# wfus/Fully-Homomorphic-Image-Processing

Hardware: AMD Instinct MI355X
Metric: encrypted 8x8 blocks/sec (homomorphic DCT+quant) (higher is better)
Workload: dtype f64

## Files before the change

fully-homomorphic-image-processing_amd/csrc/dct_fused.hip:

```cpp
#include "internal.h"

#include <cstdlib>

#include "fp64_core.h"

#pragma clang fp contract(off)

namespace {
using namespace fp64;

template <int L, int LE> struct Shape {
    static constexpr int N = 1 << L, E = 1 << LE, TP = N >> LE, NP = (L + LE - 1) / LE, LDS_WORDS = N + (N >> LE);
};
__host__ __device__ constexpr int g_lo(int L, int LE, int p) { return (L - LE * p - LE) < 0 ? 0 : (L - LE * p - LE); }
__host__ __device__ constexpr int g_stages(int L, int LE, int p) { return (L - LE * p) > LE ? LE : (L - LE * p); }
template <int LO, int LE> __device__ __forceinline__ int g_index(int tid, int r) {
    return ((tid >> LO) << (LO + LE)) | (r << LO) | (tid & ((1 << LO) - 1));
}
template <int LO, int LE> __device__ __forceinline__ int g_pad(int j) { return j + ((j >> (LO + LE)) << LO); }

template <int L, int LE, int P> struct PassTw {
    static constexpr int LO = g_lo(L, LE, P), S = g_stages(L, LE, P), NTW = (1 << LE) - 1;
    static constexpr int rb(int u) { return (L - 1 - (LE * P + u)) - LO; }
    static constexpr int count(int u) { return 1 << (LE - 1 - rb(u)); }
    static constexpr int offset(int u) { int o = 0; for (int v = 0; v < u; v++) o += count(v); return o; }
};
template <int L, int LE, int P>
__device__ __forceinline__ void load_tw(double (&w)[(1 << LE) - 1], const double *__restrict__ tw, int tid) {
    using T = PassTw<L, LE, P>;
    const int th = (P == 0) ? 0 : (tid >> T::LO);
#pragma unroll
    for (int u = 0; u < T::S; u++) {
#pragma unroll
        for (int i = 0; i < T::count(u); i++) w[T::offset(u) + i] = tw[(1 << (LE * P + u)) + ((th << (LE - 1 - T::rb(u))) | i)];
    }
}

template <int L, int LE, int P, int M>
__device__ __forceinline__ void fwd_pass(double (&x)[M][1 << LE], const double (&w)[(1 << LE) - 1], double p, double pinv) {
    using T = PassTw<L, LE, P>;
    constexpr int E = 1 << LE, KB = (LE == 3) ? 2 : 1;
#pragma unroll
    for (int u = 0; u < T::S; u++) {
        const int rb = T::rb(u);
#pragma unroll
        for (int b0 = 0; b0 < E / 2; b0 += KB) {
            double t[KB * M], wm[KB * M];
#pragma unroll
            for (int kb = 0; kb < KB; kb++) {
                const int b = b0 + kb, r0 = ((b >> rb) << (rb + 1)) | (b & ((1 << rb) - 1)), r1 = r0 | (1 << rb);
                const double wv = w[T::offset(u) + (r0 >> (rb + 1))];
#pragma unroll
                for (int m = 0; m < M; m++) { t[kb * M + m] = x[m][r1]; wm[kb * M + m] = wv; }
            }
            mmv<KB * M>(t, wm, p, pinv);
#pragma unroll
            for (int kb = 0; kb < KB; kb++) {
                const int b = b0 + kb, r0 = ((b >> rb) << (rb + 1)) | (b & ((1 << rb) - 1)), r1 = r0 | (1 << rb);
#pragma unroll
                for (int m = 0; m < M; m++) {
                    const double X = x[m][r0];
                    x[m][r0] = X + t[kb * M + m];
                    x[m][r1] = X - t[kb * M + m];
                }
            }
        }
    }
}

template <int L, int LE, int P, int M>
__device__ __forceinline__ void inv_pass(double (&x)[M][1 << LE], const double (&w)[(1 << LE) - 1], double ninv, double p, double pinv) {
    using T = PassTw<L, LE, P>;
    constexpr int E = 1 << LE, KB = (LE == 3) ? 2 : 1;
#pragma unroll
    for (int u = T::S - 1; u >= 0; u--) {
        const int sigma = LE * P + u, rb = T::rb(u);
        if (sigma == 0) {
#pragma unroll
            for (int b = 0; b < E / 2; b++) {
                const int r0 = ((b >> rb) << (rb + 1)) | (b & ((1 << rb) - 1)), r1 = r0 | (1 << rb);
                const double wv = w[T::offset(u) + (r0 >> (rb + 1))];
                double t[2 * M], wm[2 * M];
#pragma unroll
                for (int m = 0; m < M; m++) {
                    const double X = x[m][r0], Y = x[m][r1];
                    t[m] = X + Y; wm[m] = ninv;
                    t[M + m] = X - Y; wm[M + m] = wv;
                }
                mmv<2 * M>(t, wm, p, pinv);
#pragma unroll
                for (int m = 0; m < M; m++) { x[m][r0] = t[m]; x[m][r1] = t[M + m]; }
            }
        } else {
#pragma unroll
            for (int b0 = 0; b0 < E / 2; b0 += KB) {
                double t[KB * M], wm[KB * M];
#pragma unroll
                for (int kb = 0; kb < KB; kb++) {
                    const int b = b0 + kb, r0 = ((b >> rb) << (rb + 1)) | (b & ((1 << rb) - 1)), r1 = r0 | (1 << rb);
                    const double wv = w[T::offset(u) + (r0 >> (rb + 1))];
#pragma unroll
                    for (int m = 0; m < M; m++) {
                        const double X = x[m][r0], Y = x[m][r1];
                        x[m][r0] = X + Y;
                        t[kb * M + m] = X - Y; wm[kb * M + m] = wv;
                    }
                }
                mmv<KB * M>(t, wm, p, pinv);
#pragma unroll
                for (int kb = 0; kb < KB; kb++) {
                    const int b = b0 + kb, r0 = ((b >> rb) << (rb + 1)) | (b & ((1 << rb) - 1)), r1 = r0 | (1 << rb);
#pragma unroll
                    for (int m = 0; m < M; m++) x[m][r1] = t[kb * M + m];
                }
            }
        }
    }
}

template <int L, int LE, int LO_FROM, int LO_TO, int M>
__device__ __forceinline__ void transpose(double (&x)[M][1 << LE], double *lds, int tid, int &phase) {
    constexpr int PL = imin(LO_FROM, LO_TO), E = 1 << LE;
    constexpr bool WAVE_LOCAL = (Shape<L, LE>::TP <= 64) || (LO_FROM <= 6 && LO_TO <= 6);
#pragma unroll
    for (int m = 0; m < M; m++) {
        double *buf = lds + (phase & 1) * Shape<L, LE>::LDS_WORDS;
        phase++;
#pragma unroll
        for (int r = 0; r < E; r++) buf[g_pad<PL, LE>(g_index<LO_FROM, LE>(tid, r))] = x[m][r];
        if constexpr (WAVE_LOCAL) {
            __builtin_amdgcn_fence(__ATOMIC_RELEASE, "wavefront");
            __builtin_amdgcn_wave_barrier();
            __builtin_amdgcn_fence(__ATOMIC_ACQUIRE, "wavefront");
        } else {
            __syncthreads();
        }
#pragma unroll
        for (int r = 0; r < E; r++) x[m][r] = buf[g_pad<PL, LE>(g_index<LO_TO, LE>(tid, r))];
    }
}

template <int L, int LE, int M, typename PRE, int P = 0>
__device__ __forceinline__ void ntt_fwd(double (&x)[M][1 << LE], double (&w)[(1 << LE) - 1], const double *__restrict__ tw, double p, double pinv,
                                        double *lds, int tid, int &phase, PRE pre) {
    if constexpr (P + 1 < Shape<L, LE>::NP) {
        double wn[(1 << LE) - 1];
        if (LE >= 4) load_tw<L, LE, P + 1>(wn, tw, tid);
        fwd_pass<L, LE, P, M>(x, w, p, pinv);
        if (LE < 4) load_tw<L, LE, P + 1>(wn, tw, tid);
        if constexpr (P + 2 == Shape<L, LE>::NP) pre();
        transpose<L, LE, g_lo(L, LE, P), g_lo(L, LE, P + 1), M>(x, lds, tid, phase);
        ntt_fwd<L, LE, M, PRE, P + 1>(x, wn, tw, p, pinv, lds, tid, phase, pre);
    } else {
        fwd_pass<L, LE, P, M>(x, w, p, pinv);
    }
}
template <int L, int LE, int M, bool BIG, int P = Shape<L, LE>::NP - 1>
__device__ __forceinline__ void ntt_inv(double (&x)[M][1 << LE], double (&w)[(1 << LE) - 1], const double *__restrict__ itw, double p, double pinv,
                                        double *lds, int tid, int &phase) {
    if constexpr (P > 0) {
        double wn[(1 << LE) - 1];
        if (LE >= 4) load_tw<L, LE, P - 1>(wn, itw, tid);
        inv_pass<L, LE, P, M>(x, w, 0.0, p, pinv);
        if (LE < 4) load_tw<L, LE, P - 1>(wn, itw, tid);
        if constexpr (BIG) {
#pragma unroll
            for (int m = 0; m < M; m++)
#pragma unroll
                for (int r = 0; r < (1 << LE); r++) x[m][r] = red(x[m][r], p, pinv);
        }
        transpose<L, LE, g_lo(L, LE, P), g_lo(L, LE, P - 1), M>(x, lds, tid, phase);
        ntt_inv<L, LE, M, BIG, P - 1>(x, wn, itw, p, pinv, lds, tid, phase);
    } else {
        inv_pass<L, LE, P, M>(x, w, itw[0], p, pinv);
    }
}

constexpr double PACK_BIAS = 6755399441055744.0;
template <int E, int TP>
__device__ __forceinline__ void store_packed(char *__restrict__ ob, u32 vo, u32 so, const double (&x)[E]) {
    static_assert(E == 8, "packed layout is defined for 8 values per thread");
    u32 lo[8], hi[8];
#pragma unroll
    for (int r = 0; r < 8; r++) {
        const double t = x[r] + PACK_BIAS;
        lo[r] = (u32)__double2loint(t);
        hi[r] = (u32)__double2hiint(t);
    }
    u32 h[2];
#pragma unroll
    for (int g = 0; g < 2; g++) {
        const u32 p01 = __builtin_amdgcn_perm(hi[4 * g + 1], hi[4 * g + 0], 0x0c0c0400u);
        const u32 p23 = __builtin_amdgcn_perm(hi[4 * g + 3], hi[4 * g + 2], 0x0c0c0400u);
        h[g] = __builtin_amdgcn_perm(p23, p01, 0x05040100u);
    }
#pragma unroll
    for (int q = 0; q < 4; q++) *(u64 *)(ob + (size_t)(so + (q >> 1) * TP * 16 + (q & 1) * 8) + 2 * vo) = (u64)lo[2 * q] | ((u64)lo[2 * q + 1] << 32);
    *(u64 *)(ob + (size_t)(so + 4 * TP * 8) + vo) = (u64)h[0] | ((u64)h[1] << 32);
}
typedef __attribute__((address_space(3))) void lc_lptr;
template <int NT>
__device__ __forceinline__ void stage_consts(gwin_t w, u32 voff, u32 soff, u32 cstride_bytes, double *stg) {
#pragma unroll
    for (int i0 = 0; i0 < NT; i0 += 2) {
        const int i = (i0 + 1 < NT) ? i0 : NT - 2;
        __builtin_amdgcn_raw_ptr_buffer_load_lds(w, (lc_lptr *)(stg + i * 64), 16, voff, soff + (u32)i * cstride_bytes, 0, 0);
    }
}

template <int L, int LE, bool BIG, int HALF, bool PACK, bool LDSC>
__device__ __forceinline__ void rows_body(const u64 *__restrict__ in, double *__restrict__ mid, const double *__restrict__ consts,
                                          const double *__restrict__ tw, const Work &wk, double p, double pinv, u32 k, double *lds) {
    using SH = Shape<L, LE>;
    constexpr int N = SH::N, TP = SH::TP, E = SH::E, NC = HalfC<HALF>::NC, FIRST = HalfC<HALF>::FIRST;
    const int tid = threadIdx.x;
    const size_t poly_words = (size_t)k * N, ct_words = 2 * poly_words;
    const size_t base = ((size_t)wk.blk * 64 + 8 * wk.line) * ct_words + (size_t)wk.poly * poly_words + (size_t)wk.prime * N;
    const gwin_t win_in = gwin(in + base), win_mid = gwin(mid + base);
    const u32 vo = (u32)tid * 8u, ctb = (u32)(ct_words * 8);
    double w0[E - 1];
    load_tw<L, LE, 0>(w0, tw, tid);
    double x[4][E];
    u64 ra[2][E], rb[2][E];
    auto issue = [&](int m) {
#pragma unroll
        for (int r = 0; r < E; r++) {
            ra[m & 1][r] = gld_u64(win_in, vo, (u32)m * ctb + r * TP * 8);
            rb[m & 1][r] = gld_u64(win_in, vo, (u32)(7 - m) * ctb + r * TP * 8);
        }
    };
    auto combine = [&](int m) {
#pragma unroll
        for (int r = 0; r < E; r++) {
            const u64 A = ra[m & 1][r], B = rb[m & 1][r];
            x[m][r] = HALF ? u52_biased(A) - u52_biased(B) : u52_to_f64(A + B);
        }
    };
    if constexpr (LE >= 4) {
        issue(0);
        issue(1);
        asm volatile("" ::: "memory");
        combine(0);
        issue(2);
        asm volatile("" ::: "memory");
        combine(1);
        issue(3);
        asm volatile("" ::: "memory");
        combine(2);
        combine(3);
    } else {
#pragma unroll
        for (int m = 0; m < 4; m++) {
            issue(m);
            combine(m);
            asm volatile("" ::: "memory");
        }
    }
    const size_t cstride = (size_t)k * N;
    const gwin_t win_c = gwin(consts + (size_t)FIRST * cstride + (size_t)wk.prime * N);
    const u32 csb = (u32)(cstride * 8);
    double cn[9];
    auto fetch = [&](int r) {
#pragma unroll
        for (int i = 0; i < NC; i++) cn[i] = gld_f64(win_c, vo, (u32)i * csb + r * TP * 8);
    };
    int phase = 0;
    ntt_fwd<L, LE, 4>(x, w0, tw, p, pinv, lds, tid, phase, [&] { if (LE >= 4) fetch(0); });
    const int lane = tid & 63;
    double *stg = lds + (tid >> 6) * (2 * NC * 64);
    const u32 svoff = (u32)(((size_t)(lane >> 5) * cstride + (tid & ~63) + 2 * (lane & 31)) * sizeof(double));
    constexpr int NDMA = (NC + 1) / 2;
    if constexpr (LDSC) {
        __builtin_amdgcn_sched_barrier(0);
        __syncthreads();
        stage_consts<NC>(win_c, svoff, 0, csb, stg);
    }
#pragma unroll
    for (int r = 0; r < E; r++) {
        double c[9];
        if constexpr (LDSC) {
            if (r + 1 < E) stage_consts<NC>(win_c, svoff, (r + 1) * TP * 8, csb, stg + ((r + 1) & 1) * NC * 64);
            if (r + 1 < E) asm volatile("s_waitcnt vmcnt(%0)" ::"n"(NDMA) : "memory");
            else asm volatile("s_waitcnt vmcnt(0)" ::: "memory");
            const double *sr = stg + (r & 1) * NC * 64 + lane;
#pragma unroll
            for (int i = 0; i < NC; i++) c[i] = sr[i * 64];
        } else {
        if (LE < 4) fetch(r);
#pragma unroll
        for (int i = 0; i < NC; i++) c[i] = cn[i];
        if (LE >= 4 && r + 1 < E) fetch(r + 1);
        }
        line_half<HALF>(x[0][r], x[1][r], x[2][r], x[3][r], c, p, pinv);
        if (BIG) {
#pragma unroll
            for (int m = 0; m < 4; m++) x[m][r] = red(x[m][r], p, pinv);
        } else if (PACK && HALF == 0) {
            x[0][r] = red(x[0][r], p, pinv);
            x[2][r] = red(x[2][r], p, pinv);
        }
        if constexpr (LDSC) asm volatile("" ::"v"(x[0][r]), "v"(x[1][r]), "v"(x[2][r]), "v"(x[3][r]) : "memory");
    }
#pragma unroll
    for (int m = 0; m < 4; m++) {
        const u32 so = (u32)(2 * m + HALF) * ctb;
        if constexpr (PACK) {
            store_packed<E, TP>((char *)(mid + base), vo, so, x[m]);
        } else {
            if constexpr (LE >= 4) {
#pragma unroll
                for (int r = 0; r < E; r++) gst_f64(win_mid, 2 * vo, so + (r >> 1) * TP * 16 + (r & 1) * 8, x[m][r]);
            } else {
#pragma unroll
                for (int j = 0; j < E / 2; j++) gst_f64x2(win_mid, 2 * vo, so + j * TP * 16, x[m][2 * j], x[m][2 * j + 1]);
            }
        }
    }
}

__host__ __device__ constexpr int occ_waves(int tp, int lds_words) {
    return ((2 * lds_words * 16 <= 160 * 1024) ? 2 : 1) * tp / 256 < 1 ? 1 : ((2 * lds_words * 16 <= 160 * 1024) ? 2 : 1) * tp / 256;
}
template <int L, int LE> struct Occ { static constexpr int W = occ_waves(Shape<L, LE>::TP, Shape<L, LE>::LDS_WORDS); };

template <int L, int LE, bool BIG, bool PACK, bool LDSC>
__global__ __launch_bounds__((Shape<L, LE>::TP), (Occ<L, LE>::W)) void k_dct_rows(const u64 *__restrict__ in, double *__restrict__ mid,
                                                                  const double *__restrict__ consts, const double *__restrict__ tw_all,
                                                                  const Modulus *__restrict__ mods, u32 k) {
    __shared__ double lds[2 * Shape<L, LE>::LDS_WORDS];
    const Work wk = decode(blockIdx.x, k);
    const double p = (double)mods[wk.prime].q, pinv = 1.0 / p;
    const double *tw = tw_all + (size_t)wk.prime * Shape<L, LE>::N;
    if (wk.half) rows_body<L, LE, BIG, 1, PACK, LDSC>(in, mid, consts, tw, wk, p, pinv, k, lds);
    else rows_body<L, LE, BIG, 0, PACK, LDSC>(in, mid, consts, tw, wk, p, pinv, k, lds);
}

template <int L, int LE, bool BIG, int HALF, bool PACK>
__device__ __forceinline__ void cols_body(const double *__restrict__ mid, u64 *__restrict__ out, const double *__restrict__ consts,
                                          const double *__restrict__ cpairs, const double *__restrict__ itw, const Work &wk, double p, double pinv, u32 k, double *lds) {
    using SH = Shape<L, LE>;
    constexpr int N = SH::N, TP = SH::TP, E = SH::E, NC = HalfC<HALF>::NC, FIRST = HalfC<HALF>::FIRST;
    constexpr int LASTP = SH::NP - 1;
    const int tid = threadIdx.x;
    const size_t poly_words = (size_t)k * N, ct_words = 2 * poly_words;
    const size_t base = ((size_t)wk.blk * 64 + wk.line) * ct_words + (size_t)wk.poly * poly_words + (size_t)wk.prime * N;
    const size_t cstride = (size_t)k * N;
    const gwin_t win_mid = gwin(mid + base), win_out = gwin(out + base);
    const gwin_t win_c = PACK ? gwin(cpairs + 2 * ((size_t)(HALF ? 1 : 0) * cstride + (size_t)wk.prime * N))
                              : gwin(consts + (size_t)FIRST * cstride + (size_t)wk.prime * N);
    const gwin_t win_s = PACK ? gwin(cpairs + 2 * ((size_t)(DCT_NPAIR_LINE + 2 * (2 * wk.line + HALF)) * cstride + (size_t)wk.prime * N))
                              : gwin(consts + (size_t)(12 + 8 * HALF + wk.line) * cstride + (size_t)wk.prime * N);
    const gwin_t win_1 = gwin(consts + (size_t)(FIRST + NC - 1) * cstride + (size_t)wk.prime * N);
    const u32 vo = (u32)tid * 8u, rsb = (u32)(ct_words * 64), csb = (u32)(cstride * 8);
    const double pbias = p + 4503599627370496.0;
    double cn[9], sn[4];
    auto fetch = [&](int r) {
        if constexpr (PACK) {
#pragma unroll
            for (int i = 0; i < NC / 2; i++) {
                const f64x2 v = gld_f64x2(win_c, 2 * vo, (u32)i * 2 * csb + r * TP * 16);
                cn[2 * i] = v.a;
                cn[2 * i + 1] = v.b;
            }
            cn[NC - 1] = gld_f64(win_1, vo, r * TP * 8);
#pragma unroll
            for (int g = 0; g < 2; g++) {
                const f64x2 v = gld_f64x2(win_s, 2 * vo, (u32)g * 2 * csb + r * TP * 16);
                sn[2 * g] = v.a;
                sn[2 * g + 1] = v.b;
            }
        } else {
#pragma unroll
            for (int i = 0; i < NC; i++) cn[i] = gld_f64(win_c, vo, (u32)i * csb + r * TP * 8);
#pragma unroll
            for (int m = 0; m < 4; m++) sn[m] = gld_f64(win_s, vo, (u32)(16 * m) * csb + r * TP * 8);
        }
    };
    double wl[E - 1];
    if constexpr (!PACK) {
        fetch(0);
        load_tw<L, LE, LASTP>(wl, itw, tid);
    }
    double x[4][E];
    if constexpr (PACK) {
        u32x4 qa[4][2], qb[4][2];
        u64 ha[4], hb[4];
#pragma unroll
        for (int m = 0; m < 4; m++) {
#pragma unroll
            for (int g = 0; g < 2; g++) {
                qa[m][g] = gld_b128(win_mid, 2 * vo, (u32)m * rsb + g * TP * 16);
                qb[m][g] = gld_b128(win_mid, 2 * vo, (u32)(7 - m) * rsb + g * TP * 16);
            }
            ha[m] = gld_u64(win_mid, vo, (u32)m * rsb + 4 * TP * 8);
            hb[m] = gld_u64(win_mid, vo, (u32)(7 - m) * rsb + 4 * TP * 8);
        }
#pragma unroll
        for (int m = 0; m < 4; m++) {
#pragma unroll
            for (int r = 0; r < E; r++) {
                const u32 hwa = (r & 4) ? (u32)(ha[m] >> 32) : (u32)ha[m], hwb = (r & 4) ? (u32)(hb[m] >> 32) : (u32)hb[m];
                const double ta = __hiloint2double((int)(0x43380000u + (u32)(int)(signed char)(hwa >> (8 * (r & 3)))), (int)qa[m][r >> 2][r & 3]);
                const double tb = __hiloint2double((int)(0x43380000u + (u32)(int)(signed char)(hwb >> (8 * (r & 3)))), (int)qb[m][r >> 2][r & 3]);
                x[m][r] = HALF ? ta - tb : ta + (tb - 2.0 * PACK_BIAS);
            }
        }
    } else {
#pragma unroll
        for (int m = 0; m < 4; m++) {
#pragma unroll
            for (int j = 0; j < E / 2; j++) {
                const f64x2 A = gld_f64x2(win_mid, 2 * vo, (u32)m * rsb + j * TP * 16), B = gld_f64x2(win_mid, 2 * vo, (u32)(7 - m) * rsb + j * TP * 16);
                x[m][2 * j] = HALF ? A.a - B.a : A.a + B.a;
                x[m][2 * j + 1] = HALF ? A.b - B.b : A.b + B.b;
            }
        }
    }
#pragma unroll
    for (int r = 0; r < E; r++) {
        double c[9], sc[4];
        if (PACK) fetch(r);
#pragma unroll
        for (int i = 0; i < NC; i++) c[i] = cn[i];
#pragma unroll
        for (int m = 0; m < 4; m++) sc[m] = sn[m];
        if (!PACK && r + 1 < E) fetch(r + 1);
        line_half<HALF>(x[0][r], x[1][r], x[2][r], x[3][r], c, p, pinv);
        double y[4] = {x[0][r], x[1][r], x[2][r], x[3][r]};
        mmv<4>(y, sc, p, pinv);
#pragma unroll
        for (int m = 0; m < 4; m++) x[m][r] = y[m];
    }
    if constexpr (PACK) load_tw<L, LE, LASTP>(wl, itw, tid);
    int phase = 0;
    ntt_inv<L, LE, 4, BIG>(x, wl, itw, p, pinv, lds, tid, phase);
#pragma unroll
    for (int m = 0; m < 4; m++) {
#pragma unroll
        for (int r = 0; r < E; r++) gst_u64(win_out, vo, (u32)(2 * m + HALF) * rsb + r * TP * 8, f64_to_residue(x[m][r], pbias));
    }
}

template <int L, int LE, bool BIG, bool PACK>
__global__ __launch_bounds__((Shape<L, LE>::TP), (Occ<L, LE>::W)) void k_dct_cols(const double *__restrict__ mid, u64 *__restrict__ out,
                                                                  const double *__restrict__ consts, const double *__restrict__ cpairs, const double *__restrict__ itw_all,
                                                                  const Modulus *__restrict__ mods, u32 k) {
    __shared__ double lds[2 * Shape<L, LE>::LDS_WORDS];
    const Work wk = decode(blockIdx.x, k);
    const double p = (double)mods[wk.prime].q, pinv = 1.0 / p;
    const double *itw = itw_all + (size_t)wk.prime * Shape<L, LE>::N;
    if (wk.half) cols_body<L, LE, BIG, 1, PACK>(mid, out, consts, cpairs, itw, wk, p, pinv, k, lds);
    else cols_body<L, LE, BIG, 0, PACK>(mid, out, consts, cpairs, itw, wk, p, pinv, k, lds);
}

template <int L, int LE>
__global__ __launch_bounds__((Shape<L, LE>::TP), (Occ<L, LE>::W)) void k_dct_one_launch(const u64 *__restrict__ in, double *__restrict__ mid, u64 *__restrict__ out,
                                                                        const double *__restrict__ consts, const double *__restrict__ cpairs, const double *__restrict__ tw_all,
                                                                        const double *__restrict__ itw_all, const Modulus *__restrict__ mods, u32 k,
                                                                        u32 n_blocks, u32 dist, u32 *__restrict__ arrived, u32 *__restrict__ err) {
    __shared__ double lds[2 * Shape<L, LE>::LDS_WORDS];
    const u32 xcd = blockIdx.x & 7, seq = blockIdx.x >> 3, chunk = seq >> 5, r = seq & 31;
    const bool is_row = r < 16;
    const long j = is_row ? (long)chunk : (long)chunk - (long)(dist & 0xffffu);
    const u32 n_units = n_blocks * 2 * k;
    if (j < 0) return;
    const u64 g = (u64)j * 8 + xcd;
    if (g >= n_units) return;
    Work wk;
    wk.prime = (u32)(g / (n_blocks * 2));
    const u32 rem = (u32)(g - (u64)wk.prime * n_blocks * 2);
    wk.blk = rem >> 1;
    wk.poly = rem & 1;
    wk.line = (r & 15) >> 1;
    wk.half = r & 1;
    const double p = (double)mods[wk.prime].q, pinv = 1.0 / p;
    if (is_row) {
        const double *tw = tw_all + (size_t)wk.prime * Shape<L, LE>::N;
        if (wk.half) rows_body<L, LE, false, 1, true, true>(in, mid, consts, tw, wk, p, pinv, k, lds);
        else rows_body<L, LE, false, 0, true, true>(in, mid, consts, tw, wk, p, pinv, k, lds);
        if (dist & 0x10000u) return;
        __syncthreads();
        if (threadIdx.x == 0) {
            __threadfence();
            atomicAdd(arrived + g, 1u);
        }
    } else {
        if (!(dist & 0x10000u) && threadIdx.x == 0) {
            u32 spins = 0;
            while (__hip_atomic_load(arrived + g, __ATOMIC_RELAXED, __HIP_MEMORY_SCOPE_AGENT) < 16u) {
                __builtin_amdgcn_s_sleep(8);
                if (++spins > (1u << 24)) { atomicExch(err, 1u); break; }
            }
            __threadfence();
        }
        __syncthreads();
        const double *itw = itw_all + (size_t)wk.prime * Shape<L, LE>::N;
        if (wk.half) cols_body<L, LE, false, 1, true>(mid, out, consts, cpairs, itw, wk, p, pinv, k, lds);
        else cols_body<L, LE, false, 0, true>(mid, out, consts, cpairs, itw, wk, p, pinv, k, lds);
    }
}

__global__ void k_consts_to_f64(const ulonglong2 *__restrict__ in, double *__restrict__ out, const Modulus *__restrict__ mods, u32 k, u32 n, u32 le, u32 total) {
    const u32 i = blockIdx.x * blockDim.x + threadIdx.x;
    if (i >= total) return;
    const u32 pos = i % n, rowbase = i - pos;
    const u32 tp = n >> le, r = pos / tp, t = pos % tp;
    const u32 j = (t << le) + r;
    const u32 src = (j & 15) * (n >> 4) + (j >> 4);
    const u64 q = mods[(i / n) % k].q;
    const u64 w = in[rowbase + src].x;
    out[i] = w > q / 2 ? -(double)(q - w) : (double)w;
}

__global__ void k_consts_to_pairs(const ulonglong2 *__restrict__ in, double *__restrict__ out, const Modulus *__restrict__ mods, u32 k, u32 n, u32 le, u32 total) {
    const u32 i = blockIdx.x * blockDim.x + threadIdx.x;
    if (i >= total) return;
    const u32 pos = i % n, prime = (i / n) % k, pt = i / (n * k);
    const u32 tp = n >> le, r = pos / tp, t = pos % tp;
    const u32 j = (t << le) + r;
    const u32 src = (j & 15) * (n >> 4) + (j >> 4);
    u32 ca, cb;
    if (pt < DCT_NPAIR_LINE) {
        ca = pt ? 2 * pt + 1 : 0;
        cb = ca + 1;
    } else {
        const u32 u = pt - DCT_NPAIR_LINE, g = u & 1, half = (u >> 1) & 1, col = u >> 2;
        ca = 12 + 8 * (4 * g + half) + col;
        cb = ca + 16;
    }
    const u64 q = mods[prime].q;
    const u64 wa = in[((size_t)ca * k + prime) * n + src].x, wb = in[((size_t)cb * k + prime) * n + src].x;
    out[2 * (size_t)i] = wa > q / 2 ? -(double)(q - wa) : (double)wa;
    out[2 * (size_t)i + 1] = wb > q / 2 ? -(double)(q - wb) : (double)wb;
}

template <int L, int LE>
__global__ __launch_bounds__((Shape<L, LE>::TP), (Occ<L, LE>::W)) void k_rgb2ycc_f64(u64 *__restrict__ R, u64 *__restrict__ G, u64 *__restrict__ Bc,
                                                                     const double *__restrict__ consts, const double *__restrict__ tw_all,
                                                                     const double *__restrict__ itw_all, const Modulus *__restrict__ mods,
                                                                     const u64 *__restrict__ yoff, u32 yoff_len, u32 k, u32 group, u64 gstride) {
    using SH = Shape<L, LE>;
    constexpr int N = SH::N, TP = SH::TP, E = SH::E, LASTP = SH::NP - 1;
    __shared__ double lds[2 * SH::LDS_WORDS];
    const int tid = threadIdx.x;
    const u32 per_prime = gridDim.x / k;
    const u32 prime = blockIdx.x / per_prime;
    const u32 pp = blockIdx.x - prime * per_prime;
    const u32 poly = pp & 1, pix = pp >> 1;
    const u64 q = mods[prime].q;
    const double p = (double)q, pinv = 1.0 / p;
    const double *tw = tw_all + (size_t)prime * N, *itw = itw_all + (size_t)prime * N;
    const size_t pix_off = group ? (size_t)(pix / group) * gstride + (size_t)(pix % group) * 2 * k * N : (size_t)pix * 2 * k * N;
    const size_t off = pix_off + ((size_t)poly * k + prime) * N + tid;
    double w0[E - 1];
    load_tw<L, LE, 0>(w0, tw, tid);
    double x[3][E];
    {
        const u64 *src[3] = {R + off, G + off, Bc + off};
#pragma unroll
        for (int m = 0; m < 3; m++)
#pragma unroll
            for (int r = 0; r < E; r++) x[m][r] = u52_to_f64(src[m][r * TP]);
    }
    int phase = 0;
    ntt_fwd<L, LE, 3>(x, w0, tw, p, pinv, lds, tid, phase, [] {});
    double wl[E - 1];
    load_tw<L, LE, LASTP>(wl, itw, tid);
    const double *cp = consts + (size_t)prime * N + tid;
    const size_t cstride = (size_t)k * N;
#pragma unroll
    for (int r = 0; r < E; r++) {
        double c[9], y[9];
#pragma unroll
        for (int i = 0; i < 9; i++) { c[i] = cp[(size_t)i * cstride + r * TP]; y[i] = x[i % 3][r]; }
        mmv<9>(y, c, p, pinv);
        x[0][r] = y[0] + y[1] + y[2];
        x[1][r] = y[3] - y[4] + y[5];
        x[2][r] = y[6] - y[7] - y[8];
    }
    ntt_inv<L, LE, 3, false>(x, wl, itw, p, pinv, lds, tid, phase);
    u64 *dst[3] = {R + off, G + off, Bc + off};
#pragma unroll
    for (int m = 0; m < 3; m++)
#pragma unroll
// ... 58 lines not shown
        return;
    }
    double wl[E - 1];
    load_tw<L, LE, LASTP>(wl, itw, tid);
    if constexpr (MODE == 2) {
        const ulonglong2 *pp = plain + (size_t)prime * N + slot0;
#pragma unroll
        for (int r = 0; r < E; r++) {
            const double w = u52_to_f64(pp[r * (N >> 4)].x);
            double y[M], wm[M];
#pragma unroll
            for (int m = 0; m < M; m++) { y[m] = x[m][r]; wm[m] = w; }
            mmv<M>(y, wm, p, pinv);
#pragma unroll
            for (int m = 0; m < M; m++) x[m][r] = y[m];
        }
    }
    ntt_inv<L, LE, M, false>(x, wl, itw, p, pinv, lds, tid, phase);
#pragma unroll
    for (int m = 0; m < M; m++) {
        u64 *dst = out + ((size_t)(g * M + m) * k + prime) * N + tid;
#pragma unroll
        for (int r = 0; r < E; r++) {
            double v = x[m][r];
            v = v < 0.0 ? v + p : v;
            dst[r * TP] = f64_to_u52(v);
        }
    }
}

}


static u32 dct_shape_le(const fhe_ctx *c) {
    if (c->opt.dct_le != 3) return 4;
    if (c->logn == 12 && c->max_prime_bits <= 40) return 3;
    if (c->logn == 13 || c->logn == 11) return 3;
    return 4;
}

bool fhe_dct_f64_supported(const fhe_ctx *c) {
    return c && c->qb.d_tw_f64 && c->max_prime_bits <= 47 && (c->logn >= 10 && c->logn <= 13);
}

int fhe_dct_f64_make_consts(const fhe_ctx *c, fhe_dct_plan *plan, hipStream_t st) {
    const u32 total = DCT_NCONST * c->k * c->n, pairs = DCT_NPAIR * c->k * c->n;
    const u32 le = dct_shape_le(c);
    const bool packed = c->max_prime_bits <= 37 && le == 3 && c->opt.dct_pack;
    HIP_TRY(hipMalloc(&plan->d_consts_f64, sizeof(double) * total));
    if (packed) { HIP_TRY(hipMalloc(&plan->d_consts_pair, 2 * sizeof(double) * pairs)); }
    k_consts_to_f64<<<(total + 255) / 256, 256, 0, st>>>(plan->d_consts, plan->d_consts_f64, c->qb.d_mod, c->k, c->n, le, total);
    KERNEL_CHECK();
    if (packed) {
        k_consts_to_pairs<<<(pairs + 255) / 256, 256, 0, st>>>(plan->d_consts, plan->d_consts_pair, c->qb.d_mod, c->k, c->n, le, pairs);
        KERNEL_CHECK();
    }
    return FHE_OK;
}



template <int L, int LE>
static void launch_pair(const fhe_ctx *c, const fhe_dct_plan *plan, const u64 *in, u64 *out, double *mid, unsigned grid, bool big, hipStream_t st, int which) {
    constexpr int TP = Shape<L, LE>::TP;
    if constexpr (LE == 4) {
        if (big) {
            if (which & 1) k_dct_rows<L, LE, true, false, false><<<grid, TP, 0, st>>>(in, mid, plan->d_consts_f64, c->qb.d_tw_f64, c->qb.d_mod, c->k);
            if (which & 2) k_dct_cols<L, LE, true, false><<<grid, TP, 0, st>>>(mid, out, plan->d_consts_f64, plan->d_consts_pair, c->qb.d_itw_f64, c->qb.d_mod, c->k);
            return;
        }
    }
    if constexpr (LE == 3) {
        if (big) {
            if (which & 1) k_dct_rows<L, LE, true, false, false><<<grid, TP, 0, st>>>(in, mid, plan->d_consts_f64, c->qb.d_tw_f64, c->qb.d_mod, c->k);
            if (which & 2) k_dct_cols<L, LE, true, false><<<grid, TP, 0, st>>>(mid, out, plan->d_consts_f64, plan->d_consts_pair, c->qb.d_itw_f64, c->qb.d_mod, c->k);
            return;
        }
        if (c->max_prime_bits <= 37 && c->opt.dct_pack) {
            if (which & 1) {
                if (c->opt.dct_ldsc) k_dct_rows<L, LE, false, true, true><<<grid, TP, 0, st>>>(in, mid, plan->d_consts_f64, c->qb.d_tw_f64, c->qb.d_mod, c->k);
                else k_dct_rows<L, LE, false, true, false><<<grid, TP, 0, st>>>(in, mid, plan->d_consts_f64, c->qb.d_tw_f64, c->qb.d_mod, c->k);
            }
            if (which & 2) k_dct_cols<L, LE, false, true><<<grid, TP, 0, st>>>(mid, out, plan->d_consts_f64, plan->d_consts_pair, c->qb.d_itw_f64, c->qb.d_mod, c->k);
            return;
        }
    }
    {
        if (which & 1) k_dct_rows<L, LE, false, false, false><<<grid, TP, 0, st>>>(in, mid, plan->d_consts_f64, c->qb.d_tw_f64, c->qb.d_mod, c->k);
        if (which & 2) k_dct_cols<L, LE, false, false><<<grid, TP, 0, st>>>(mid, out, plan->d_consts_f64, plan->d_consts_pair, c->qb.d_itw_f64, c->qb.d_mod, c->k);
    }
}

int fhe_dct_f64_launch(const fhe_ctx *c, const fhe_dct_plan *plan, const u64 *in, u64 *out, u64 n_blocks, double *mid, hipStream_t st, int which) {
    const u64 items = n_blocks * 8 * 2 * c->k;
    const u64 grid = items * 2;
    if (grid > 0x7fffffffULL) return fail(FHE_ERR_PARAM, "too many blocks for one launch");
    if ((u64)c->k * c->n >= (1ULL << 21)) return fail(FHE_ERR_PARAM, "fused FP64 path: a block of ciphertexts exceeds the 2 GiB addressing window");
    const bool big = c->max_prime_bits > 40;
    if (!big && dct_shape_le(c) == 3 && c->max_prime_bits <= 37 && c->opt.dct_pack && !plan->d_consts_pair)
        return fail(FHE_ERR_PARAM, "fused FP64 path: the plan has no paired constant tables (it was created for a context without the packed intermediate)");
    if (c->opt.dct_one_launch && which == 3 && c->logn == 12 && dct_shape_le(c) == 3 && c->max_prime_bits <= 37 && c->opt.dct_pack && c->d_arrived) {
        const u64 n_units = n_blocks * 2 * c->k;
        if (n_units > c->arrived_cap) return fail(FHE_ERR_PARAM, "one-launch experiment: wave too large for the arrival counters");
        HIP_TRY(hipMemsetAsync(c->d_arrived, 0, (n_units + 1) * sizeof(u32), st));
        const u32 dist = c->opt.dct_one_launch;
        const u64 chunks = (n_units + 7) / 8 + (dist & 0xffffu);
        k_dct_one_launch<12, 3><<<(unsigned)(chunks * 32 * 8), Shape<12, 3>::TP, 0, st>>>(in, mid, out, plan->d_consts_f64, plan->d_consts_pair, c->qb.d_tw_f64, c->qb.d_itw_f64, c->qb.d_mod,
                                                                                       c->k, (u32)n_blocks, dist, c->d_arrived + 1, c->d_arrived);
        KERNEL_CHECK();
        u32 timed_out = 0;
        HIP_TRY(hipMemcpyAsync(&timed_out, c->d_arrived, sizeof(u32), hipMemcpyDeviceToHost, st));
        HIP_TRY(hipStreamSynchronize(st));
        if (timed_out) return fail(FHE_ERR_HIP, "one-launch experiment: a column workgroup timed out waiting for its row transforms; the output is incomplete");
        return FHE_OK;
    }
    switch (c->logn) {
        case 10: launch_pair<10, 4>(c, plan, in, out, mid, (unsigned)grid, big, st, which); break;
        case 11: launch_pair<11, 3>(c, plan, in, out, mid, (unsigned)grid, big, st, which); break;
        case 12: if (dct_shape_le(c) == 3) launch_pair<12, 3>(c, plan, in, out, mid, (unsigned)grid, false, st, which); else launch_pair<12, 4>(c, plan, in, out, mid, (unsigned)grid, big, st, which); break;
        case 13: if (dct_shape_le(c) == 3) launch_pair<13, 3>(c, plan, in, out, mid, (unsigned)grid, big, st, which); else launch_pair<13, 4>(c, plan, in, out, mid, (unsigned)grid, big, st, which); break;
        default: return fail(FHE_ERR_PARAM, "fused FP64 path supports n in {1024, 2048, 4096, 8192}");
    }
    KERNEL_CHECK();
    return FHE_OK;
}

bool fhe_rgb_f64_supported(const fhe_ctx *c) {
    return fhe_dct_f64_supported(c) && c->logn == 12 && c->max_prime_bits <= 40;
}

int fhe_rgb_f64_make_consts(const fhe_ctx *c, const ulonglong2 *d_c, double **out, hipStream_t st) {
    const u32 total = 9 * c->k * c->n;
    HIP_TRY(hipMalloc(out, sizeof(double) * total));
    k_consts_to_f64<<<(total + 255) / 256, 256, 0, st>>>(d_c, *out, c->qb.d_mod, c->k, c->n, 3, total);
    KERNEL_CHECK();
    return FHE_OK;
}

int fhe_rgb_f64_launch(const fhe_ctx *c, u64 *r, u64 *g, u64 *b, u64 count, const double *consts, const u64 *yoff, u32 yoff_len, hipStream_t st, u32 group, u64 gstride) {
    const u64 grid = count * 2 * c->k;
    if (grid > 0x7fffffffULL) return fail(FHE_ERR_PARAM, "too many pixels for one launch");
    k_rgb2ycc_f64<12, 3><<<(unsigned)grid, Shape<12, 3>::TP, 0, st>>>(r, g, b, consts, c->qb.d_tw_f64, c->qb.d_itw_f64, c->qb.d_mod, yoff, yoff_len, c->k, group, gstride);
// ... 193 lines not shown
```

fully-homomorphic-image-processing_amd/csrc/internal.h:

```cpp
#pragma once
#include "../../include/fhe_hip.h"

#include <hip/hip_runtime.h>

#include <mutex>
#include <string>
#include <vector>

#include "modarith.h"
#include "ntt_core.h"

int fhe_fail(int code, const char *fmt, ...) __attribute__((format(printf, 2, 3)));
#define fail fhe_fail
#define HIP_TRY(expr)                                                                             \
    do {                                                                                          \
        hipError_t e_ = (expr);                                                                   \
        if (e_ != hipSuccess) return fail(FHE_ERR_HIP, "%s: %s", #expr, hipGetErrorString(e_));   \
    } while (0)
#define KERNEL_CHECK()                                                                            \
    do {                                                                                          \
        hipError_t e_ = hipGetLastError();                                                        \
        if (e_ != hipSuccess) return fail(FHE_ERR_HIP, "kernel launch: %s", hipGetErrorString(e_)); \
    } while (0)

// ... 22 lines not shown
    bool ntt_nolazy = false;
    bool ntt_single = false;
    bool ntt_nopm = false;
    bool behz_aux61 = false;
    bool behz_chunk3 = false;
    bool behz_tensor_canon = false;
    bool behz_tensor_single = false;
    bool behz_square_full = false;
    bool plain_sum_unfused = false;
    bool cubic_unfused = false;
    bool enc_unfused = false;
    bool enc_occ4 = false;
    bool relin_steps = false;
    bool relin_fused = false;
    bool filter_xcd = true;
    bool galois_staged = false;
    bool galois_gather_lds = false;
    bool behz_fused_prepare = false;
};

struct fhe_ctx {
    u32 n = 0, logn = 0, k = 0;
    FheOptions opt;
    u64 t = 0;
    int device = 0;
    int max_prime_bits = 0;
    BaseTables qb;
    u64 upper_half_threshold = 0;
    u64 plain_upper_half_increment[FHE_MAX_K] = {0};
    u64 delta_mod[FHE_MAX_K] = {0};
    u64 upper_half_increment[FHE_MAX_K] = {0};
    struct BehzTables *behz = nullptr;
    mutable std::once_flag behz_once;
    int behz_rc = 0;
    std::string behz_err;
    u32 *d_arrived = nullptr;
    u64 arrived_cap = 0;
    hipStream_t aux_stream = nullptr;
    hipEvent_t ev_rows[2] = {nullptr, nullptr}, ev_cols[2] = {nullptr, nullptr};
    struct RgbConsts {
        int int_coeffs = -1, frac_coeffs = -1;
        ulonglong2 *d_c = nullptr;
        double *d_c_f64 = nullptr;
        u64 *d_off = nullptr;
        u32 off_len = 0;
    };
    mutable std::vector<RgbConsts *> rgb;
    mutable std::vector<RgbConsts *> ycc;
    mutable std::mutex rgb_mutex;
};

#define DCT_NCONST 76
#define DCT_NPAIR_LINE 5
#define DCT_NPAIR (DCT_NPAIR_LINE + 32)
extern const double kDctConst[12];
struct fhe_dct_plan {
    ulonglong2 *d_consts = nullptr;
    double *d_consts_f64 = nullptr;
    double *d_consts_pair = nullptr;
    ulonglong2 *d_consts_le3 = nullptr;
    u32 k = 0, n = 0;
    bool has_quant = false;
};

inline float fhe_resize_ref_coord(u32 i, u32 dst_len, u32 src_len) { return (float)((float)i / (float)(dst_len - 1) * (float)src_len - 0.5); }

#define DISPATCH_L(logn, ...)                                                    \
    switch (logn) {                                                              \
        case 10: { constexpr int L = 10; __VA_ARGS__; } break;                   \
        case 11: { constexpr int L = 11; __VA_ARGS__; } break;                   \
        case 12: { constexpr int L = 12; __VA_ARGS__; } break;                   \
        case 13: { constexpr int L = 13; __VA_ARGS__; } break;                   \
        case 14: { constexpr int L = 14; __VA_ARGS__; } break;                   \
        default: return fail(FHE_ERR_PARAM, "unsupported log2(n)=%u", logn);     \
    }

struct CMap {
    const u32 *idx;
    u64 div, cnt, off;
    __device__ __forceinline__ u64 operator()(u64 c) const { return idx ? idx[c] : (cnt ? ((off + c / div) % cnt) : c); }
};

#define FHE_PLAIN_SUM_MAX_TERMS 16
struct PlainSumTerms {
    u32 count;
    u32 size[FHE_PLAIN_SUM_MAX_TERMS];
    u64 *src[FHE_PLAIN_SUM_MAX_TERMS];
    const ulonglong2 *plain[FHE_PLAIN_SUM_MAX_TERMS];
};
bool fhe_multiply_plain_sum_supported(const fhe_ctx *c);
int fhe_multiply_plain_sum(const fhe_ctx *c, const PlainSumTerms &T, const u64 *addend, CMap amap, u32 addend_size, u64 *out, u32 out_size, u64 count,
                           hipStream_t st);

#define FHE_STAGE_SLOT_BYTES ((size_t)256 << 10)
struct FheStage { void *dev; int slot; void *ring; };
int fhe_stage_acquire(const void *host, size_t bytes, hipStream_t st, FheStage *out);
int fhe_stage_release(const FheStage &sg, hipStream_t st);
int fhe_ntt_launch(bool inverse, const fhe_ctx *c, const BaseTables &B, const u64 *in, u64 *out, u64 n_res_polys, hipStream_t st);
int fhe_build_base(BaseTables &B, const std::vector<u64> &primes, u32 n, u32 logn, bool want_f64);
void fhe_free_base(BaseTables &B);
int fhe_behz_build(fhe_ctx *c);
int fhe_behz_ensure(const fhe_ctx *c);
bool fhe_behz_floor3_supported(const fhe_ctx *c);
size_t fhe_behz_d_words(const fhe_ctx *c, u32 so, u64 count);
int fhe_behz_tensor_shared(const fhe_ctx *c, const u64 *a, u32 sa, const u64 *bp, u32 sb, u64 b_count, u64 b_div, u64 b_first, u64 *d, u64 count,
                           u64 *scratch, hipStream_t st);
int fhe_behz_floor3_combine(const fhe_ctx *c, const u64 *da, const u64 *db, const u64 *dc, u32 size_ab, u32 size_c, const u64 *B, CMap mB, u32 size_b,
// ... 18 lines not shown
```

Baseline: 88620.

## Fold DCT column constants and inverse-NTT scaling into precomputed pair tables

Adds four compile-time options, all on by default, to the packed column DCT kernel. P1 always uses the pipelined row-load schedule. P2 prefetches the scale constants one row ahead. P3 folds the inverse-NTT n^-1 factor into the constant pairs so the final butterfly skips one multiply. P4 precomputes the even-half line DCT products into six-wide scale constants, which removes the line_half multiply step and the cn loads. The aim is fewer modular multiplies and fewer constant loads per element, at the cost of a larger constant table, more registers, and a new sigma-0 path that must keep numerical correctness.

Result: slower. 60410 (-31.8%).

```diff
diff --git a/fully-homomorphic-image-processing_amd/csrc/dct_fused.hip b/fully-homomorphic-image-processing_amd/csrc/dct_fused.hip
--- a/fully-homomorphic-image-processing_amd/csrc/dct_fused.hip
+++ b/fully-homomorphic-image-processing_amd/csrc/dct_fused.hip
@@ -5,6 +5,19 @@
 #include "fp64_core.h"
 
 #pragma clang fp contract(off)
+
+#ifndef DCT_P1
+#define DCT_P1 1
+#endif
+#ifndef DCT_P2
+#define DCT_P2 1
+#endif
+#ifndef DCT_P3
+#define DCT_P3 1
+#endif
+#ifndef DCT_P4
+#define DCT_P4 1
+#endif
 
 namespace {
 using namespace fp64;
@@ -68,14 +81,36 @@
     }
 }
 
-template <int L, int LE, int P, int M>
+template <int L, int LE, int P, int M, bool FOLD = false>
 __device__ __forceinline__ void inv_pass(double (&x)[M][1 << LE], const double (&w)[(1 << LE) - 1], double ninv, double p, double pinv) {
     using T = PassTw<L, LE, P>;
     constexpr int E = 1 << LE, KB = (LE == 3) ? 2 : 1;
 #pragma unroll
     for (int u = T::S - 1; u >= 0; u--) {
         const int sigma = LE * P + u, rb = T::rb(u);
-        if (sigma == 0) {
+        if (sigma == 0 && FOLD) {
+#pragma unroll
+            for (int b0 = 0; b0 < E / 2; b0 += KB) {
+                double t[KB * M], wm[KB * M];
+#pragma unroll
+                for (int kb = 0; kb < KB; kb++) {
+                    const int b = b0 + kb, r0 = ((b >> rb) << (rb + 1)) | (b & ((1 << rb) - 1)), r1 = r0 | (1 << rb);
+#pragma unroll
+                    for (int m = 0; m < M; m++) {
+                        const double X = x[m][r0], Y = x[m][r1];
+                        x[m][r0] = X + Y;
+                        t[kb * M + m] = X - Y; wm[kb * M + m] = ninv;
+                    }
+                }
+                mmv<KB * M>(t, wm, p, pinv);
+#pragma unroll
+                for (int kb = 0; kb < KB; kb++) {
+                    const int b = b0 + kb, r0 = ((b >> rb) << (rb + 1)) | (b & ((1 << rb) - 1)), r1 = r0 | (1 << rb);
+#pragma unroll
+                    for (int m = 0; m < M; m++) { x[m][r0] = red(x[m][r0], p, pinv); x[m][r1] = t[kb * M + m]; }
+                }
+            }
+        } else if (sigma == 0) {
 #pragma unroll
             for (int b = 0; b < E / 2; b++) {
                 const int r0 = ((b >> rb) << (rb + 1)) | (b & ((1 << rb) - 1)), r1 = r0 | (1 << rb);
@@ -155,9 +190,9 @@
         fwd_pass<L, LE, P, M>(x, w, p, pinv);
     }
 }
-template <int L, int LE, int M, bool BIG, int P = Shape<L, LE>::NP - 1>
+template <int L, int LE, int M, bool BIG, int P = Shape<L, LE>::NP - 1, bool FOLD = false>
 __device__ __forceinline__ void ntt_inv(double (&x)[M][1 << LE], double (&w)[(1 << LE) - 1], const double *__restrict__ itw, double p, double pinv,
-                                        double *lds, int tid, int &phase) {
+                                        double *lds, int tid, int &phase, double w1 = 0.0) {
     if constexpr (P > 0) {
         double wn[(1 << LE) - 1];
         if (LE >= 4) load_tw<L, LE, P - 1>(wn, itw, tid);
@@ -170,9 +205,9 @@
                 for (int r = 0; r < (1 << LE); r++) x[m][r] = red(x[m][r], p, pinv);
         }
         transpose<L, LE, g_lo(L, LE, P), g_lo(L, LE, P - 1), M>(x, lds, tid, phase);
-        ntt_inv<L, LE, M, BIG, P - 1>(x, wn, itw, p, pinv, lds, tid, phase);
+        ntt_inv<L, LE, M, BIG, P - 1, FOLD>(x, wn, itw, p, pinv, lds, tid, phase, w1);
     } else {
-        inv_pass<L, LE, P, M>(x, w, itw[0], p, pinv);
+        inv_pass<L, LE, P, M, FOLD>(x, w, FOLD ? w1 : itw[0], p, pinv);
     }
 }
 
@@ -236,7 +271,7 @@
             x[m][r] = HALF ? u52_biased(A) - u52_biased(B) : u52_to_f64(A + B);
         }
     };
-    if constexpr (LE >= 4) {
+    if constexpr (LE >= 4 || DCT_P1) {
         issue(0);
         issue(1);
         asm volatile("" ::: "memory");
@@ -337,10 +372,13 @@
 
 template <int L, int LE, bool BIG, int HALF, bool PACK>
 __device__ __forceinline__ void cols_body(const double *__restrict__ mid, u64 *__restrict__ out, const double *__restrict__ consts,
-                                          const double *__restrict__ cpairs, const double *__restrict__ itw, const Work &wk, double p, double pinv, u32 k, double *lds) {
+                                          const double *__restrict__ cpairs, const double *__restrict__ itw, double w1, const Work &wk, double p, double pinv, u32 k, double *lds) {
     using SH = Shape<L, LE>;
     constexpr int N = SH::N, TP = SH::TP, E = SH::E, NC = HalfC<HALF>::NC, FIRST = HalfC<HALF>::FIRST;
     constexpr int LASTP = SH::NP - 1;
+    constexpr bool EV6 = PACK && HALF == 0 && DCT_P4, FOLD = PACK && DCT_P3;
+    constexpr int NS = EV6 ? 6 : 4;
+    constexpr bool AHEAD = PACK && (DCT_P2 == 1 || DCT_P2 == 2 || (DCT_P2 == 3 && HALF == 0));
     const int tid = threadIdx.x;
     const size_t poly_words = (size_t)k * N, ct_words = 2 * poly_words;
     const size_t base = ((size_t)wk.blk * 64 + wk.line) * ct_words + (size_t)wk.poly * poly_words + (size_t)wk.prime * N;
@@ -348,27 +386,32 @@
     const gwin_t win_mid = gwin(mid + base), win_out = gwin(out + base);
     const gwin_t win_c = PACK ? gwin(cpairs + 2 * ((size_t)(HALF ? 1 : 0) * cstride + (size_t)wk.prime * N))
                               : gwin(consts + (size_t)FIRST * cstride + (size_t)wk.prime * N);
-    const gwin_t win_s = PACK ? gwin(cpairs + 2 * ((size_t)(DCT_NPAIR_LINE + 2 * (2 * wk.line + HALF)) * cstride + (size_t)wk.prime * N))
+    const gwin_t win_s = PACK ? gwin(cpairs + 2 * ((size_t)(DCT_NPAIR_LINE + DCT_PAIR_COL(wk.line, HALF)) * cstride + (size_t)wk.prime * N))
                               : gwin(consts + (size_t)(12 + 8 * HALF + wk.line) * cstride + (size_t)wk.prime * N);
     const gwin_t win_1 = gwin(consts + (size_t)(FIRST + NC - 1) * cstride + (size_t)wk.prime * N);
     const u32 vo = (u32)tid * 8u, rsb = (u32)(ct_words * 64), csb = (u32)(cstride * 8);
     const double pbias = p + 4503599627370496.0;
-    double cn[9], sn[4];
+    double cn[9], sn[NS];
+    auto fetch_s = [&](int r) {
+#pragma unroll
+        for (int g = 0; g < NS / 2; g++) {
+            const f64x2 v = gld_f64x2(win_s, 2 * vo, (u32)g * 2 * csb + r * TP * 16);
+            sn[2 * g] = v.a;
+            sn[2 * g + 1] = v.b;
+        }
+    };
     auto fetch = [&](int r) {
         if constexpr (PACK) {
-#pragma unroll
-            for (int i = 0; i < NC / 2; i++) {
-                const f64x2 v = gld_f64x2(win_c, 2 * vo, (u32)i * 2 * csb + r * TP * 16);
-                cn[2 * i] = v.a;
-                cn[2 * i + 1] = v.b;
-            }
-            cn[NC - 1] = gld_f64(win_1, vo, r * TP * 8);
-#pragma unroll
-            for (int g = 0; g < 2; g++) {
-                const f64x2 v = gld_f64x2(win_s, 2 * vo, (u32)g * 2 * csb + r * TP * 16);
-                sn[2 * g] = v.a;
-                sn[2 * g + 1] = v.b;
-            }
+            if constexpr (!EV6) {
+#pragma unroll
+                for (int i = 0; i < NC / 2; i++) {
+                    const f64x2 v = gld_f64x2(win_c, 2 * vo, (u32)i * 2 * csb + r * TP * 16);
+                    cn[2 * i] = v.a;
+                    cn[2 * i + 1] = v.b;
+                }
+                cn[NC - 1] = gld_f64(win_1, vo, r * TP * 8);
+            }
+            if (!AHEAD) fetch_s(r);
         } else {
 #pragma unroll
             for (int i = 0; i < NC; i++) cn[i] = gld_f64(win_c, vo, (u32)i * csb + r * TP * 8);
@@ -395,6 +438,7 @@
             ha[m] = gld_u64(win_mid, vo, (u32)m * rsb + 4 * TP * 8);
             hb[m] = gld_u64(win_mid, vo, (u32)(7 - m) * rsb + 4 * TP * 8);
         }
+        if (AHEAD && DCT_P2 == 1) fetch_s(0);
 #pragma unroll
         for (int m = 0; m < 4; m++) {
 #pragma unroll
@@ -416,24 +460,42 @@
             }
         }
     }
+    if (AHEAD && DCT_P2 != 1) fetch_s(0);
 #pragma unroll
     for (int r = 0; r < E; r++) {
-        double c[9], sc[4];
+        double c[9], sc[NS];
         if (PACK) fetch(r);
-#pragma unroll
-        for (int i = 0; i < NC; i++) c[i] = cn[i];
-#pragma unroll
-        for (int m = 0; m < 4; m++) sc[m] = sn[m];
+        if constexpr (!EV6) {
+#pragma unroll
+            for (int i = 0; i < NC; i++) c[i] = cn[i];
+        }
+#pragma unroll
+        for (int m = 0; m < NS; m++) sc[m] = sn[m];
         if (!PACK && r + 1 < E) fetch(r + 1);
+        if (AHEAD && r + 1 < E) fetch_s(r + 1);
+        if constexpr (EV6) {
+            const double x0 = x[0][r], x1 = x[1][r], x2 = x[2][r], x3 = x[3][r];
+            const double tmp10 = x0 + x3, tmp13 = x0 - x3, tmp11 = x1 + x2, tmp12 = x1 - x2;
+            double y[6] = {tmp10 + tmp11, tmp10 - tmp11, tmp13, tmp12, tmp13, tmp12};
+            mmv<6>(y, sc, p, pinv);
+            x[0][r] = y[0];
+            x[2][r] = y[1];
+            x[1][r] = y[2] + y[3];
+            x[3][r] = y[4] + y[5];
+        } else {
         line_half<HALF>(x[0][r], x[1][r], x[2][r], x[3][r], c, p, pinv);
         double y[4] = {x[0][r], x[1][r], x[2][r], x[3][r]};
         mmv<4>(y, sc, p, pinv);
 #pragma unroll
         for (int m = 0; m < 4; m++) x[m][r] = y[m];
+        }
+#ifdef DCT_P2_PIN
+        if constexpr (AHEAD) asm volatile("" ::"v"(x[0][r]), "v"(x[1][r]), "v"(x[2][r]), "v"(x[3][r]) : "memory");
+#endif
     }
     if constexpr (PACK) load_tw<L, LE, LASTP>(wl, itw, tid);
     int phase = 0;
-    ntt_inv<L, LE, 4, BIG>(x, wl, itw, p, pinv, lds, tid, phase);
+    ntt_inv<L, LE, 4, BIG, LASTP, FOLD>(x, wl, itw, p, pinv, lds, tid, phase, w1);
 #pragma unroll
     for (int m = 0; m < 4; m++) {
 #pragma unroll
@@ -443,14 +505,15 @@
 
 template <int L, int LE, bool BIG, bool PACK>
 __global__ __launch_bounds__((Shape<L, LE>::TP), (Occ<L, LE>::W)) void k_dct_cols(const double *__restrict__ mid, u64 *__restrict__ out,
-                                                                  const double *__restrict__ consts, const double *__restrict__ cpairs, const double *__restrict__ itw_all,
-                                                                  const Modulus *__restrict__ mods, u32 k) {
+                                                                  const double *__restrict__ consts, const double *__restrict__ cpairs, const double *__restrict__ tw_all,
+                                                                  const double *__restrict__ itw_all, const Modulus *__restrict__ mods, u32 k) {
     __shared__ double lds[2 * Shape<L, LE>::LDS_WORDS];
     const Work wk = decode(blockIdx.x, k);
     const double p = (double)mods[wk.prime].q, pinv = 1.0 / p;
     const double *itw = itw_all + (size_t)wk.prime * Shape<L, LE>::N;
-    if (wk.half) cols_body<L, LE, BIG, 1, PACK>(mid, out, consts, cpairs, itw, wk, p, pinv, k, lds);
-    else cols_body<L, LE, BIG, 0, PACK>(mid, out, consts, cpairs, itw, wk, p, pinv, k, lds);
+    const double w1 = PACK ? -tw_all[(size_t)wk.prime * Shape<L, LE>::N + 1] : 0.0;
+    if (wk.half) cols_body<L, LE, BIG, 1, PACK>(mid, out, consts, cpairs, itw, w1, wk, p, pinv, k, lds);
+    else cols_body<L, LE, BIG, 0, PACK>(mid, out, consts, cpairs, itw, w1, wk, p, pinv, k, lds);
 }
 
 template <int L, int LE>
@@ -495,8 +558,9 @@
         }
         __syncthreads();
         const double *itw = itw_all + (size_t)wk.prime * Shape<L, LE>::N;
-        if (wk.half) cols_body<L, LE, false, 1, true>(mid, out, consts, cpairs, itw, wk, p, pinv, k, lds);
-        else cols_body<L, LE, false, 0, true>(mid, out, consts, cpairs, itw, wk, p, pinv, k, lds);
+        const double w1 = -tw_all[(size_t)wk.prime * Shape<L, LE>::N + 1];
+        if (wk.half) cols_body<L, LE, false, 1, true>(mid, out, consts, cpairs, itw, w1, wk, p, pinv, k, lds);
+        else cols_body<L, LE, false, 0, true>(mid, out, consts, cpairs, itw, w1, wk, p, pinv, k, lds);
     }
 }
 
@@ -512,24 +576,47 @@
     out[i] = w > q / 2 ? -(double)(q - w) : (double)w;
 }
 
-__global__ void k_consts_to_pairs(const ulonglong2 *__restrict__ in, double *__restrict__ out, const Modulus *__restrict__ mods, u32 k, u32 n, u32 le, u32 total) {
+__global__ void k_consts_to_pairs(const ulonglong2 *__restrict__ in, double *__restrict__ out, const ulonglong2 *__restrict__ itw, const Modulus *__restrict__ mods, u32 k, u32 n, u32 le, u32 total) {
     const u32 i = blockIdx.x * blockDim.x + threadIdx.x;
     if (i >= total) return;
     const u32 pos = i % n, prime = (i / n) % k, pt = i / (n * k);
     const u32 tp = n >> le, r = pos / tp, t = pos % tp;
     const u32 j = (t << le) + r;
     const u32 src = (j & 15) * (n >> 4) + (j >> 4);
-    u32 ca, cb;
+    const u64 q = mods[prime].q;
+    auto cst = [&](u32 cid) { return in[((size_t)cid * k + prime) * n + src]; };
+    auto mul = [&](u64 x, const ulonglong2 c) { return mul_shoup(x, c.x, c.y, q); };
+    const ulonglong2 ninv = itw[(size_t)prime * n];
+    u64 wa, wb;
     if (pt < DCT_NPAIR_LINE) {
-        ca = pt ? 2 * pt + 1 : 0;
-        cb = ca + 1;
+        const u32 ca = pt ? 2 * pt + 1 : 0;
+        wa = cst(ca).x;
+        wb = cst(ca + 1).x;
     } else {
+#if DCT_P4
+        const u32 u = pt - DCT_NPAIR_LINE, col = u / 5, e = u % 5;
+        auto scale = [&](u32 row) { return cst(12 + 8 * row + col); };
+        if (e == 1 || e == 2) {
+            const u64 c0 = cst(0).x, cx = addmod(c0, cst(e).x, q);
+            const ulonglong2 s = scale(e == 1 ? 2 : 6);
+            wa = mul(e == 1 ? cx : c0, s);
+            wb = mul(e == 1 ? c0 : cx, s);
+        } else {
+            const u32 row = e == 0 ? 0 : e == 3 ? 1 : 5;
+            wa = scale(row).x;
+            wb = scale(row + (e == 0 ? 4 : 2)).x;
+        }
+#else
         const u32 u = pt - DCT_NPAIR_LINE, g = u & 1, half = (u >> 1) & 1, col = u >> 2;
-        ca = 12 + 8 * (4 * g + half) + col;
-        cb = ca + 16;
-    }
-    const u64 q = mods[prime].q;
-    const u64 wa = in[((size_t)ca * k + prime) * n + src].x, wb = in[((size_t)cb * k + prime) * n + src].x;
+        const u32 ca = 12 + 8 * (4 * g + half) + col;
+        wa = cst(ca).x;
+        wb = cst(ca + 16).x;
+#endif
+#if DCT_P3
+        wa = mul(wa, ninv);
+        wb = mul(wb, ninv);
+#endif
+    }
     out[2 * (size_t)i] = wa > q / 2 ? -(double)(q - wa) : (double)wa;
     out[2 * (size_t)i + 1] = wb > q / 2 ? -(double)(q - wb) : (double)wb;
 }
@@ -694,7 +781,7 @@
     k_consts_to_f64<<<(total + 255) / 256, 256, 0, st>>>(plan->d_consts, plan->d_consts_f64, c->qb.d_mod, c->k, c->n, le, total);
     KERNEL_CHECK();
     if (packed) {
-        k_consts_to_pairs<<<(pairs + 255) / 256, 256, 0, st>>>(plan->d_consts, plan->d_consts_pair, c->qb.d_mod, c->k, c->n, le, pairs);
+        k_consts_to_pairs<<<(pairs + 255) / 256, 256, 0, st>>>(plan->d_consts, plan->d_consts_pair, c->qb.d_itw, c->qb.d_mod, c->k, c->n, le, pairs);
         KERNEL_CHECK();
     }
     return FHE_OK;
@@ -708,14 +795,14 @@
     if constexpr (LE == 4) {
         if (big) {
             if (which & 1) k_dct_rows<L, LE, true, false, false><<<grid, TP, 0, st>>>(in, mid, plan->d_consts_f64, c->qb.d_tw_f64, c->qb.d_mod, c->k);
-            if (which & 2) k_dct_cols<L, LE, true, false><<<grid, TP, 0, st>>>(mid, out, plan->d_consts_f64, plan->d_consts_pair, c->qb.d_itw_f64, c->qb.d_mod, c->k);
+            if (which & 2) k_dct_cols<L, LE, true, false><<<grid, TP, 0, st>>>(mid, out, plan->d_consts_f64, plan->d_consts_pair, c->qb.d_tw_f64, c->qb.d_itw_f64, c->qb.d_mod, c->k);
             return;
         }
     }
     if constexpr (LE == 3) {
         if (big) {
             if (which & 1) k_dct_rows<L, LE, true, false, false><<<grid, TP, 0, st>>>(in, mid, plan->d_consts_f64, c->qb.d_tw_f64, c->qb.d_mod, c->k);
-            if (which & 2) k_dct_cols<L, LE, true, false><<<grid, TP, 0, st>>>(mid, out, plan->d_consts_f64, plan->d_consts_pair, c->qb.d_itw_f64, c->qb.d_mod, c->k);
+            if (which & 2) k_dct_cols<L, LE, true, false><<<grid, TP, 0, st>>>(mid, out, plan->d_consts_f64, plan->d_consts_pair, c->qb.d_tw_f64, c->qb.d_itw_f64, c->qb.d_mod, c->k);
             return;
         }
         if (c->max_prime_bits <= 37 && c->opt.dct_pack) {
@@ -723,13 +810,13 @@
                 if (c->opt.dct_ldsc) k_dct_rows<L, LE, false, true, true><<<grid, TP, 0, st>>>(in, mid, plan->d_consts_f64, c->qb.d_tw_f64, c->qb.d_mod, c->k);
                 else k_dct_rows<L, LE, false, true, false><<<grid, TP, 0, st>>>(in, mid, plan->d_consts_f64, c->qb.d_tw_f64, c->qb.d_mod, c->k);
             }
-            if (which & 2) k_dct_cols<L, LE, false, true><<<grid, TP, 0, st>>>(mid, out, plan->d_consts_f64, plan->d_consts_pair, c->qb.d_itw_f64, c->qb.d_mod, c->k);
+            if (which & 2) k_dct_cols<L, LE, false, true><<<grid, TP, 0, st>>>(mid, out, plan->d_consts_f64, plan->d_consts_pair, c->qb.d_tw_f64, c->qb.d_itw_f64, c->qb.d_mod, c->k);
             return;
         }
     }
     {
         if (which & 1) k_dct_rows<L, LE, false, false, false><<<grid, TP, 0, st>>>(in, mid, plan->d_consts_f64, c->qb.d_tw_f64, c->qb.d_mod, c->k);
-        if (which & 2) k_dct_cols<L, LE, false, false><<<grid, TP, 0, st>>>(mid, out, plan->d_consts_f64, plan->d_consts_pair, c->qb.d_itw_f64, c->qb.d_mod, c->k);
+        if (which & 2) k_dct_cols<L, LE, false, false><<<grid, TP, 0, st>>>(mid, out, plan->d_consts_f64, plan->d_consts_pair, c->qb.d_tw_f64, c->qb.d_itw_f64, c->qb.d_mod, c->k);
     }
 }
 
diff --git a/fully-homomorphic-image-processing_amd/csrc/internal.h b/fully-homomorphic-image-processing_amd/csrc/internal.h
--- a/fully-homomorphic-image-processing_amd/csrc/internal.h
+++ b/fully-homomorphic-image-processing_amd/csrc/internal.h
@@ -98,7 +98,16 @@
 
 #define DCT_NCONST 76
 #define DCT_NPAIR_LINE 5
+#ifndef DCT_P4
+#define DCT_P4 1
+#endif
+#if DCT_P4
+#define DCT_NPAIR (DCT_NPAIR_LINE + 40)
+#define DCT_PAIR_COL(col, half) (5 * (col) + ((half) ? 3 : 0))
+#else
 #define DCT_NPAIR (DCT_NPAIR_LINE + 32)
+#define DCT_PAIR_COL(col, half) (2 * (2 * (col) + (half)))
+#endif
 extern const double kDctConst[12];
 struct fhe_dct_plan {
     ulonglong2 *d_consts = nullptr;
```
